# SpeakerGuard/SpeakerGuard

Hardware: AMD Instinct MI355X
Metric: PGD attack steps/sec (xv_plda, 3s@16kHz, batch 64) (higher is better)
Workload: dtype f32

## Files before the change

include/speakerguard_hip.h:

```cpp
#ifndef SPEAKERGUARD_HIP_H
#define SPEAKERGUARD_HIP_H

#include <stddef.h>
#include <stdint.h>

#ifdef __cplusplus
extern "C" {
#endif

typedef struct sg_ctx sg_ctx;

#define SG_OK 0
#define SG_ERR_ARG 1
#define SG_ERR_HIP 2
#define SG_ERR_STATE 3

int sg_version(void);
int sg_create(int device, sg_ctx** out);
void sg_destroy(sg_ctx* ctx);
const char* sg_last_error(const sg_ctx* ctx);
int sg_sync(sg_ctx* ctx, void* stream);
int sg_health(sg_ctx* ctx);
int sg_set_streamk(sg_ctx* ctx, int32_t enable);
int sg_debug_lose_handoffs(sg_ctx* ctx, int32_t launches);
// ... 136 lines not shown
} sg_an_weights;

int sg_an_load(sg_ctx* ctx, const sg_an_weights* w);
int32_t sg_an_num_frames(int32_t T);
int sg_an_logmel(sg_ctx* ctx, const float* x_dev, int32_t B, int32_t T, float* feats_dev, void* stream);
int sg_an_logmel_backward(sg_ctx* ctx, const float* x_dev, int32_t B, int32_t T, const float* dfeats_dev, float* grad_dev,
                          int32_t reuse_forward, void* stream);
int sg_an_configure(sg_ctx* ctx, int32_t fft_bits, int32_t spectrum_cache, int32_t fused_overlap_add);
int sg_an_forward(sg_ctx* ctx, const float* x_dev, int32_t B, int32_t T_or_F, int32_t flag,
                  int64_t* decisions_dev, float* scores_dev, float* emb_dev, void* stream);
int sg_an_debug_activation(sg_ctx* ctx, int32_t layer, float* out_dev, int64_t capacity_floats,
                           int32_t* rows_per_utt, int32_t* channels, void* stream);
int sg_an_loss_grad(sg_ctx* ctx, const float* x_dev, const int64_t* y_dev, int32_t B, int32_t T_or_F,
                    int32_t flag, const sg_loss_spec* loss, int64_t* decisions_dev, float* scores_dev,
                    float* loss_dev, float* grad_dev, void* stream);
int sg_an_pgd_run(sg_ctx* ctx, float* x_adv_dev, const int64_t* y_dev, const float* lower_dev,
                  const float* upper_dev, int32_t B, int32_t T, const sg_pgd_params* params,
                  uint8_t* success_dev, int64_t* decisions_dev, float* scores_dev, float* loss_dev,
                  float* loss_trace_dev, int64_t* decision_trace_dev, void* stream);

int sg_xv_time_layer(sg_ctx* ctx, int32_t layer, int32_t B, int32_t T, int32_t iters,
                     float* ms_per_launch, double* flops, int32_t* tile_rows, void* stream);

#define SG_STAGE_MFCC_FWD 10
#define SG_STAGE_CMVN_FWD 11
#define SG_STAGE_POOL_FWD 12
#define SG_STAGE_FC1_FWD 13
#define SG_STAGE_TAIL 14
#define SG_STAGE_FC1_BWD 15
#define SG_STAGE_POOL_BWD 16
#define SG_STAGE_CMVN_BWD 17
#define SG_STAGE_MFCC_BWD 18
#define SG_STAGE_OVERLAP_ADD 19
#define SG_STAGE_AN_LOGMEL_FWD 20
#define SG_STAGE_AN_PREFILTER_FWD 21
#define SG_STAGE_AN_POOL_FWD 22
#define SG_STAGE_AN_TAIL 23
#define SG_STAGE_AN_POOL_BWD 24
#define SG_STAGE_AN_PREFILTER_BWD 25
#define SG_STAGE_AN_LOGMEL_BWD 26
#define SG_STAGE_AN_OVERLAP_ADD 27
#define SG_STAGE_AN_FECO_FWD 28
#define SG_STAGE_AN_FECO_BWD 29
#define SG_STAGE_AN_CONV_FWD 30
#define SG_STAGE_AN_CONV_BWD 40
#define SG_STAGE_AN_FUSED_FWD 50
#define SG_STAGE_AN_FUSED_BWD 51
#define SG_STAGE_AN_FUSED_FWDBWD 52
int sg_trace_begin(sg_ctx* ctx, int32_t max_records);
int sg_trace_end(sg_ctx* ctx, int32_t* tags_out, float* ms_out, int32_t capacity, int32_t* n_out);

int sg_conv1d_rows(sg_ctx* ctx, const float* a_dev, const float* w_dev, float* c_dev, const float* bias_dev,
                   const float* mask_dev, int32_t B, int32_t Ta, int32_t Tc, int32_t Kc, int32_t N, int32_t taps,
                   int32_t tap_step, int32_t tap_base, int32_t epi, int32_t kernel, void* stream);

int sg_wav_finalize(sg_ctx* ctx, const float* benign_dev, const float* adver_dev, int32_t B, int32_t T,
                    int16_t* pcm_dev, double* metrics_dev, void* stream);

int sg_eer_threshold(sg_ctx* ctx, const float* target_dev, int32_t n_target, const float* untarget_dev,
                     int32_t n_untarget, double* out3_dev, void* stream);

int sg_feco_kmeans(sg_ctx* ctx, const float* feats_dev, int32_t B, int32_t F, int32_t D, int32_t k, int32_t max_iter,
                   int32_t* assign_dev, void* stream);
int sg_feco_kmeans_seeded(sg_ctx* ctx, const float* feats_dev, int32_t B, int32_t F, int32_t D, int32_t k, int32_t max_iter,
                          uint64_t seed, int64_t index_base, int32_t* assign_dev, void* stream);
int sg_feco_compress(sg_ctx* ctx, const float* feats_dev, const int32_t* assign_dev, int32_t B, int32_t F, int32_t D,
// ... 31 lines not shown
```

speakerguard_amd/_native.py:

```python
import ctypes as C
import os

_HERE = os.path.dirname(os.path.abspath(__file__))
LIB_PATH = os.path.join(_HERE, "libspeakerguard_hip.so")

SG_LOSS_ENTROPY, SG_LOSS_MARGIN, SG_LOSS_LINEAR = 0, 1, 2
SG_TASK = {"CSI": 0, "SV": 1, "OSI": 2}
SG_FLAG_WAV, SG_FLAG_RAW, SG_FLAG_CMVN = 0, 1, 2

EXPORTS = (
    "sg_version", "sg_create", "sg_destroy", "sg_last_error", "sg_sync", "sg_xv_load", "sg_xv_set_enroll",
    "sg_xv_num_frames", "sg_input_scale", "sg_xv_mfcc", "sg_xv_cmvn", "sg_xv_forward", "sg_xv_debug_activation",
    "sg_xv_loss_grad", "sg_loss_eval", "sg_pgd_update", "sg_xv_pgd_run", "sg_xv_time_layer",
    "sg_cw2_step", "sg_nes_queries", "sg_nes_grad", "sg_fakebob_step",
    "sg_an_load", "sg_an_num_frames", "sg_an_logmel", "sg_an_forward", "sg_an_debug_activation", "sg_an_loss_grad",
    "sg_an_pgd_run", "sg_an_pgd_run_feco", "sg_conv1d_rows", "sg_wav_finalize", "sg_eer_threshold",
    "sg_xv_mfcc_backward", "sg_xv_cmvn_backward", "sg_feco_kmeans", "sg_feco_kmeans_seeded", "sg_feco_kmeans_compress", "sg_feco_compress_backward_reps", "sg_feco_compress", "sg_feco_compress_backward", "sg_feco_warped",
    "sg_an_logmel_backward", "sg_an_configure", "sg_xv_configure", "sg_xv_enroll_override", "sg_health", "sg_set_streamk", "sg_debug_lose_handoffs", "sg_debug_feco_epoch", "sg_feco_set_two_cu", "sg_trace_begin", "sg_trace_end",
)

STAGE_NAMES = {10: "mfcc_fwd", 11: "cmvn_fwd", 12: "pool_fwd", 13: "fc1_fwd", 14: "tail", 15: "fc1_bwd", 16: "pool_bwd",
               17: "cmvn_bwd", 18: "mfcc_bwd", 19: "overlap_add"}
STAGE_NAMES.update({l: "tdnn%d_fwd" % l for l in range(1, 6)})
STAGE_NAMES.update({-l: "tdnn%d_dgrad" % l for l in range(1, 6)})
STAGE_NAMES.update({20: "an_logmel_fwd", 21: "an_prefilter_fwd", 22: "an_pool_fwd", 23: "an_tail", 24: "an_pool_bwd",
                    25: "an_prefilter_bwd", 26: "an_logmel_bwd", 27: "an_overlap_add", 28: "an_feco_fwd", 29: "an_feco_bwd",
                    50: "an_cnn_fwd", 51: "an_cnn_bwd", 52: "an_cnn_fwdbwd"})
STAGE_NAMES.update({30 + l: "an_conv%d_fwd" % (l + 2) for l in range(7)})
STAGE_NAMES.update({40 + l: "an_conv%d_dgrad" % (l + 2) for l in range(7)})


class NativeError(RuntimeError):
    pass


class XvWeights(C.Structure):
    _fields_ = [
        ("tdnn_weight", C.c_void_p * 5), ("tdnn_bias", C.c_void_p * 5),
        ("bn_mean", C.c_void_p * 5), ("bn_var", C.c_void_p * 5),
        ("fc1_weight", C.c_void_p), ("fc1_bias", C.c_void_p), ("emb_mean", C.c_void_p), ("lda", C.c_void_p),
        ("plda_mean", C.c_void_p), ("plda_transform", C.c_void_p), ("plda_psi", C.c_void_p), ("enroll", C.c_void_p),
        ("D", C.c_int32), ("S", C.c_int32), ("bn_eps", C.c_float), ("threshold", C.c_float),
    ]


class AnWeights(C.Structure):
    _fields_ = [
        ("conv1_weight", C.c_void_p), ("conv1_bias", C.c_void_p), ("bn1", C.c_void_p * 4),
        ("conv_weight", C.c_void_p * 7), ("conv_bias", C.c_void_p * 7), ("bn_weight", C.c_void_p * 7),
        ("bn_bias", C.c_void_p * 7), ("bn_mean", C.c_void_p * 7), ("bn_var", C.c_void_p * 7),
        ("fc_weight", C.c_void_p), ("fc_bias", C.c_void_p), ("num_class", C.c_int32), ("bn_eps", C.c_float),
    ]


class LossSpec(C.Structure):
# ... 137 lines not shown
```

speakerguard_amd/csrc/k_mfcc.hip:

```cpp
#include "sg_internal.h"
#include "fft512t.h"

namespace sg {

constexpr int kMfccMaxBlocks = 512;

template <typename R> struct MfccCfg;
#ifndef SG_MFCC_F32_WAVES
#define SG_MFCC_F32_WAVES 8
#define SG_MFCC_F32_OCC 4
#endif
template <> struct MfccCfg<float> { static constexpr int kWaves = SG_MFCC_F32_WAVES, kMinBlocks = SG_MFCC_F32_OCC; };
template <> struct MfccCfg<double> { static constexpr int kWaves = 4, kMinBlocks = 2; };

template <typename R>
struct FrameLdsT {
    cx<R> spec[kFft + kFft / 8];
    float power[256];
    float mel[32];
    float lmel[32];
    float tmp[32];
};

static_assert(kMfccTw1 == kFftTw1 && kMfccTw2 == kFftTw2, "table sizes of fft512.h");
// ... 168 lines not shown
        cep_out = v;
    }
}

template <typename R, int DZ>
__global__ __launch_bounds__(MfccCfg<R>::kWaves * 64, MfccCfg<R>::kMinBlocks) void mfcc_fwd_kernel(MfccTables t, const float* __restrict__ x, int B, int T, int F,
                                                                          const float* __restrict__ scale_p, sg_dither dz,
                                                                          float* __restrict__ feats) {
    constexpr int kWaves = MfccCfg<R>::kWaves;
    __shared__ FrameLdsT<R> lds[kWaves];
    __shared__ TabLdsT<R> tb;
    stage_tables<R>(t, tb);
    const int lane = threadIdx.x & 63, wid = threadIdx.x >> 6;
    const float scale = scale_p ? *scale_p : 1.f;
    FrameLdsT<R>& L = lds[wid];
    const int total = B * F, stride = gridDim.x * kWaves;
    float raw[7], nxt[7];
    load_frame(x, T, F, blockIdx.x * kWaves + wid, total, lane, nxt, t.rep_utts);
    for (int gf = blockIdx.x * kWaves + wid; gf < total; gf += stride) {
        const int b = gf / F, f = gf - b * F;
        const int tz = opaque_zero();
#pragma unroll
        for (int i = 0; i < 7; ++i) raw[i] = nxt[i];
        load_frame(x, T, F, gf + stride, total, lane, nxt, t.rep_utts);
        FrameState st;
        float cep;
        cx<R> Xk[4];
        frame_forward<R, 0, DZ>(t, tb, tz, L, raw, F, b, f, scale, dz, lane, st, cep, Xk);
        if (lane < kCep) feats[((size_t)b * F + f) * kCep + lane] = cep;
        wave_sync();
    }
}

template <typename R, bool CACHED, int DZ>
__global__ __launch_bounds__(MfccCfg<R>::kWaves * 64, CACHED ? MfccCfg<R>::kMinBlocks : 1) void mfcc_bwd_kernel(MfccTables t, const float* __restrict__ x, int B, int T, int F,
                                                                          const float* __restrict__ scale_p, sg_dither dz,
                                                                          const float* __restrict__ dfeats, int ld,
                                                                          float* __restrict__ dframes) {
    constexpr int kWaves = MfccCfg<R>::kWaves;
    __shared__ FrameLdsT<R> lds[kWaves];
    __shared__ TabLdsT<R> tb;
    stage_tables<R>(t, tb);
    const int lane = threadIdx.x & 63, wid = threadIdx.x >> 6;
    const float scale = scale_p ? *scale_p : 1.f;
    FrameLdsT<R>& L = lds[wid];
    const int kb = (lane >> 3) + 8 * (lane & 7);
    int bin_m0[4];
    float bin_w0[4], bin_w1[4];
#pragma unroll
    for (int d = 0; d < 4; ++d) {
        bin_m0[d] = t.bin_m0[kb + 64 * d];
        bin_w0[d] = t.bin_w0[kb + 64 * d];
        bin_w1[d] = t.bin_w1[kb + 64 * d];
    }
    const int total = B * F, stride = gridDim.x * kWaves;
    float raw[7], nxt[7];
    load_frame(x, T, F, blockIdx.x * kWaves + wid, total, lane, nxt, t.rep_utts);
    for (int gf = blockIdx.x * kWaves + wid; gf < total; gf += stride) {
        const int b = gf / F, f = gf - b * F;
        const int tz = opaque_zero();
#pragma unroll
        for (int i = 0; i < 7; ++i) raw[i] = nxt[i];
        load_frame(x, T, F, gf + stride, total, lane, nxt, t.rep_utts);
        FrameState st;
        float cep;
        cx<R> Xk[4];
        frame_forward<R, CACHED ? 1 : 0, DZ>(t, tb, tz, L, raw, F, b, f, scale, dz, lane, st, cep, Xk);
        float dc = 0.f;
        if (lane < kCep) dc = dfeats[((size_t)b * F + f) * ld + lane];
        const float denergy = __shfl(dc, 0, 64);
        if (lane < 32) L.tmp[lane] = (lane == 0 || lane >= kCep) ? 0.f : dc * tb.lifter[lane];
        wave_sync();
        if (lane < 32) {
            float dm = 0.f;
            if (lane < kMel) {
                float dl = 0.f;
#pragma unroll
                for (int c = 0; c < kCep; ++c) dl = __builtin_fmaf(L.tmp[c], tb.dct_t[tz + c * 32 + lane], dl);
                const float mel = L.mel[lane];
                dm = mel > kEps ? dl / mel : 0.f;
            }
            L.lmel[lane] = dm;
        }
        wave_sync();
        cx<R> v[8];
#pragma unroll
        for (int d = 0; d < 4; ++d) {
            v[d] = cmk<R>((R)0, (R)0);
            const int m0 = bin_m0[d];
            if (m0 >= 0) {
                const R dp = (R)(2.f * __builtin_fmaf(L.lmel[m0], bin_w0[d], L.lmel[m0 + 1] * bin_w1[d]));
                v[d] = cmk<R>(Xk[d].x * dp, Xk[d].y * dp);
            }
        }
#pragma unroll
        for (int d = 4; d < 8; ++d) v[d] = cmk<R>((R)0, (R)0);
        fft512T_transposed<R>(L.spec, tb.tw1c() + tz, tb.tw2c() + tz, lane, (R)1, v);
        float sw[8];
#pragma unroll
        for (int i = 0; i < 7; ++i) sw[i] = (float)v[i].x * tb.window[tz + lane + 64 * i];
        sw[7] = 0.f;
        float ds[7];
        float sum = 0.f;
        const float einv = st.energy > kEps ? 2.f * denergy / st.energy : 0.f;
#pragma unroll
        for (int i = 0; i < 7; ++i) {
            const int n = lane + 64 * i;
            const float edge = __builtin_bit_cast(float, __builtin_amdgcn_readlane(__builtin_bit_cast(int, sw[i + 1]), 0));
            const float next = __builtin_bit_cast(float, __builtin_amdgcn_update_dpp(__builtin_bit_cast(int, edge), __builtin_bit_cast(int, sw[i]),
                                                                                      0x130 , 0xf, 0xf, false));
            float g = 0.f;
            if (n < kWin) {
                g = sw[i] - 0.97f * next;
                if (n == 0) g -= 0.97f * sw[0];
                g = __builtin_fmaf(einv, st.s[i], g);
            }
            ds[i] = g;
            sum += g;
        }
        const float mean = wave_sum(sum) / (float)kWin;
#pragma unroll
        for (int i = 0; i < 7; ++i) {
            const int n = lane + 64 * i;
            if (n < kWin) dframes[((size_t)b * F + f) * kWin + n] = (ds[i] - mean) * scale;
        }
        wave_sync();
    }
}
#pragma clang fp contract(fast)

template <int V>
__global__ __launch_bounds__(256) void frames_to_wave_kernel(const float* __restrict__ dframes, int B, int T, int F, int R,
                                                             const float* acc_in, float* grad_out, float* __restrict__ x_io,
                                                             const float* __restrict__ lower,
                                                             const float* __restrict__ upper, float step, int grad_sign) {
    const int n0 = (blockIdx.x * 256 + threadIdx.x) * V;
    const int b = blockIdx.y;
    if (n0 >= T) return;
    constexpr int kPad = kWin / 2 - kShift / 2;
    const int last_q = (F - 1) * kShift - kPad + kWin - 1;
    const size_t o = (size_t)b * T + n0;
    float total[V];
    const bool interior = V == 4 && n0 >= kPad && 2 * T - 1 - (n0 + 3) > last_q && n0 + 3 < T;
    if (interior) {
        typedef float f4 __attribute__((ext_vector_type(4)));
        const int q = n0 + kPad;
        int fhi = q / kShift;
        const int flo = q > kWin - 1 ? (q - (kWin - 1) + kShift - 1) / kShift : 0;
        if (fhi > F - 1) fhi = F - 1;
        f4 tot = {0.f, 0.f, 0.f, 0.f};
        for (int r = 0; r < R; ++r) {
            const float* df = dframes + ((size_t)r * B + b) * F * kWin;
            f4 g = {0.f, 0.f, 0.f, 0.f};
            for (int f = flo; f <= fhi; ++f) g += *reinterpret_cast<const f4*>(df + (size_t)f * kWin + (q - f * kShift));
            if (r == 0) tot = acc_in ? *reinterpret_cast<const f4*>(acc_in + o) + g : g;
            else tot = tot + g;
        }
// ... 25 lines not shown
        }
    }
    if (V == 4 && n0 + 3 < T) {
        typedef float f4 __attribute__((ext_vector_type(4)));
        if (grad_out) *reinterpret_cast<f4*>(grad_out + o) = f4{total[0], total[V > 1 ? 1 : 0], total[V > 2 ? 2 : 0], total[V > 3 ? 3 : 0]};
        if (x_io) {
            const f4 xv = *reinterpret_cast<const f4*>(x_io + o), lo = *reinterpret_cast<const f4*>(lower + o),
                     hi = *reinterpret_cast<const f4*>(upper + o);
            f4 res;
#pragma unroll
            for (int v = 0; v < 4; ++v) {
                const float g = total[v < V ? v : 0];
                const float sg = g > 0.f ? 1.f : (g < 0.f ? -1.f : 0.f);
                res[v] = fminf(fmaxf(xv[v] + step * sg * (float)grad_sign, lo[v]), hi[v]);
            }
            *reinterpret_cast<f4*>(x_io + o) = res;
        }
        return;
    }
#pragma unroll
    for (int v = 0; v < V; ++v) {
        if (n0 + v >= T) break;
        const float g = total[v];
        if (grad_out) grad_out[o + v] = g;
        if (x_io) {
            const float sg = g > 0.f ? 1.f : (g < 0.f ? -1.f : 0.f);
            float val = x_io[o + v] + step * sg * (float)grad_sign;
            val = fminf(fmaxf(val, lower[o + v]), upper[o + v]);
            x_io[o + v] = val;
        }
    }
}

template <typename R>
static void mfcc_fwd_launch(const MfccTables& t, const float* x, int B, int T, int F, const float* scale, const sg_dither& d,
                            float* feats, hipStream_t s) {
    constexpr int kWaves = MfccCfg<R>::kWaves;
    const int want = (B * F + kWaves - 1) / kWaves;
    dim3 grid(want < kMfccMaxBlocks ? want : kMfccMaxBlocks);
    if (d.noise_dev) hipLaunchKernelGGL((mfcc_fwd_kernel<R, 2>), grid, dim3(kWaves * 64), 0, s, t, x, B, T, F, scale, d, feats);
    else if (d.dither != 0.f) hipLaunchKernelGGL((mfcc_fwd_kernel<R, 1>), grid, dim3(kWaves * 64), 0, s, t, x, B, T, F, scale, d, feats);
    else hipLaunchKernelGGL((mfcc_fwd_kernel<R, 0>), grid, dim3(kWaves * 64), 0, s, t, x, B, T, F, scale, d, feats);
}

template <typename R>
static void mfcc_bwd_launch(const MfccTables& t, const float* x, int B, int T, int F, const float* scale, const sg_dither& d,
                            const float* dfeats, float* dframes, hipStream_t s) {
    constexpr int kWaves = MfccCfg<R>::kWaves;
    const int want = (B * F + kWaves - 1) / kWaves;
    dim3 grid(want < kMfccMaxBlocks ? want : kMfccMaxBlocks);
#define SG_MFCC_BWD(CACHED, DZ) \
    hipLaunchKernelGGL((mfcc_bwd_kernel<R, CACHED, DZ>), grid, dim3(kWaves * 64), 0, s, t, x, B, T, F, scale, d, dfeats, kCep, dframes)
    const int dzk = d.noise_dev ? 2 : (d.dither != 0.f ? 1 : 0);
    if (t.spec_cache) {
        if (dzk == 2) SG_MFCC_BWD(true, 2); else if (dzk == 1) SG_MFCC_BWD(true, 1); else SG_MFCC_BWD(true, 0);
    } else {
        if (dzk == 2) SG_MFCC_BWD(false, 2); else if (dzk == 1) SG_MFCC_BWD(false, 1); else SG_MFCC_BWD(false, 0);
    }
#undef SG_MFCC_BWD
}

hipError_t launch_mfcc_fwd(const MfccTables& t, const float* x, int B, int T, int F, const float* scale,
                           const sg_dither* dz, float* feats, hipStream_t s) {
    sg_dither d = dz ? *dz : sg_dither{0.f, 0, 0, nullptr};
    if (t.fft64) mfcc_fwd_launch<double>(t, x, B, T, F, scale, d, feats, s);
    else mfcc_fwd_launch<float>(t, x, B, T, F, scale, d, feats, s);
    return hipGetLastError();
}

hipError_t launch_mfcc_bwd(const MfccTables& t, const float* x, int B, int T, int F, const float* scale,
                           const sg_dither* dz, const float* dfeats, float* dframes, hipStream_t s) {
    sg_dither d = dz ? *dz : sg_dither{0.f, 0, 0, nullptr};
    if (t.fft64) mfcc_bwd_launch<double>(t, x, B, T, F, scale, d, dfeats, dframes, s);
    else mfcc_bwd_launch<float>(t, x, B, T, F, scale, d, dfeats, dframes, s);
    return hipGetLastError();
}

hipError_t launch_frames_to_wave(const float* dframes, int B, int T, int F, int R, const float* acc_in, float* grad_out,
                                 float* x_io, const float* lower, const float* upper, float step, int grad_sign,
                                 hipStream_t s) {
    const uintptr_t bases = reinterpret_cast<uintptr_t>(grad_out) | reinterpret_cast<uintptr_t>(x_io) |
                            reinterpret_cast<uintptr_t>(lower) | reinterpret_cast<uintptr_t>(upper) |
                            reinterpret_cast<uintptr_t>(acc_in) | reinterpret_cast<uintptr_t>(dframes);
    if (T % 4 == 0 && bases % 16 == 0 && (long)B * T >= 16L * 48000) {
        dim3 grid((T / 4 + 255) / 256, B);
        hipLaunchKernelGGL(frames_to_wave_kernel<4>, grid, dim3(256), 0, s, dframes, B, T, F, R, acc_in, grad_out, x_io, lower, upper,
                           step, grad_sign);
    } else {
        dim3 grid((T + 255) / 256, B);
        hipLaunchKernelGGL(frames_to_wave_kernel<1>, grid, dim3(256), 0, s, dframes, B, T, F, R, acc_in, grad_out, x_io, lower, upper,
                           step, grad_sign);
    }
    return hipGetLastError();
}

}
```

speakerguard_amd/csrc/sg_api.hip:

```cpp
#include <algorithm>
#include <cmath>
#include <cstdarg>
#include <cstdio>
#include <cstdlib>
#include <cstring>
#include <memory>
#include <type_traits>

#include "sg_internal.h"

using namespace sg;

namespace {

int fail(sg_ctx* ctx, int code, const char* fmt, ...) {
    char buf[512];
    va_list ap;
    va_start(ap, fmt);
    vsnprintf(buf, sizeof(buf), fmt, ap);
    va_end(ap);
    if (ctx) ctx->err = buf;
    return code;
}

// ... 343 lines not shown
    if (int h = sg_health(ctx)) return h;
    SG_HIP(hipSetDevice(ctx->device));
    if (B < 1) return fail(ctx, SG_ERR_ARG, "B must be >= 1");
    if (flag < 0 || flag > 2) return fail(ctx, SG_ERR_ARG, "flag must be 0 (wav), 1 (raw feat) or 2 (cmvn feat)");
    d->B = B;
    if (flag == SG_FLAG_WAV) {
        if (TF < kWin) return fail(ctx, SG_ERR_ARG, "waveform shorter than one 25 ms window");
        d->T = TF;
        d->F = num_frames(TF);
    } else {
        d->T = 0;
        d->F = TF;
    }
    int Fl[kLayers];
    if (!layer_frames(d->F, Fl)) return fail(ctx, SG_ERR_ARG, "%d frames are too few for the TDNN context", d->F);
    {
        size_t worst = 0;
        for (int l = 0; l < kLayers; ++l) {
            const size_t bytes = (size_t)B * Fl[l] * kCoutPad[l] * sizeof(float);
            if (bytes > worst) worst = bytes;
        }
        if (worst >= 0x80000000ull)
            return fail(ctx, SG_ERR_ARG, "batch of %d x %d frames needs a %.1f GiB activation tensor; one pass handles < 2 GiB "
                        "(at most %d utterances of this length): split the batch", B, d->F, (double)worst / (1ull << 30),
                        (int)(0x7FFFFFFFull / (worst / (size_t)B)));
    }
    int rc = build_tables(ctx);
    if (rc) return rc;
    rc = ensure_workspace(ctx, d->B, d->T, d->F);
    if (rc) return fail(ctx, rc, "workspace allocation failed: %s", ctx->err.c_str());
    return SG_OK;
}

int run_backward_to_input(sg_ctx* ctx, const float* x, const PassDims& d, int flag, const sg_dither* dz,
                          float* grad_out, float* x_update, const float* lower, const float* upper, float step,
                          int grad_sign, hipStream_t s, const float* grad_acc_in = nullptr) {
    Workspace& w = ctx->ws;
    int rc = run_tdnn_backward(ctx, d, s);
    if (rc) return rc;
    if (flag == SG_FLAG_CMVN) {
        SG_HIP(launch_sum_cols(w.dfeats, kFeatPad, kL1BwdSplitK, (long long)d.B * d.F * kFeatPad, grad_out, kCep,
                               (int64_t)d.B * d.F, kCep, s));
    } else if (flag == SG_FLAG_RAW) {
        SG_HIP(launch_cmvn_bwd(w.dfeats, kFeatPad, kL1BwdSplitK, (long long)d.B * d.F * kFeatPad, grad_out, kCep, d.B,
                               d.F, s));
    } else {
        SG_STAGE(SG_STAGE_CMVN_BWD, launch_cmvn_bwd(w.dfeats, kFeatPad, kL1BwdSplitK, (long long)d.B * d.F * kFeatPad,
                                                    w.dfeats_raw, kCep, d.B, d.F, s));
        MfccTables tab = ctx->tab;
        static const bool use_cache = [] {
            const char* e = sg_tune_env("SG_MFCC_CACHE");
            return !e || atoi(e) != 0;
        }();
        if (use_cache) {
            tab.spec_cache = w.spec_cache;
            tab.mel_cache = w.mel_cache;
        }
        tab.rep_utts = d.Bu;
        const int utts = d.Bu > 0 ? d.Bu : d.B;
        SG_STAGE(SG_STAGE_MFCC_BWD, launch_mfcc_bwd(tab, x, d.B, d.T, d.F, w.scale, dz, w.dfeats_raw, w.dframes, s));
        SG_STAGE(SG_STAGE_OVERLAP_ADD, launch_frames_to_wave(w.dframes, utts, d.T, d.F, d.B / utts, grad_acc_in, grad_out, x_update,
                                                             lower, upper, step, grad_sign, s));
    }
    return SG_OK;
}

}

extern "C" {

int sg_version(void) { return 100; }

int sg_create(int device, sg_ctx** out) {
    if (!out) return SG_ERR_ARG;
    *out = nullptr;
    int n = 0;
    if (hipGetDeviceCount(&n) != hipSuccess || device < 0 || device >= n) return SG_ERR_HIP;
    if (hipSetDevice(device) != hipSuccess) return SG_ERR_HIP;
    sg_ctx* ctx = new (std::nothrow) sg_ctx();
    if (!ctx) return SG_ERR_HIP;
    ctx->device = device;
    hipDeviceProp_t prop;
    if (hipGetDeviceProperties(&prop, device) == hipSuccess && prop.multiProcessorCount > 0)
        ctx->num_cus = prop.multiProcessorCount;
    if (hipEventCreate(&ctx->ev0) != hipSuccess || hipEventCreate(&ctx->ev1) != hipSuccess) {
        delete ctx;
        return SG_ERR_HIP;
// ... 413 lines not shown
        const int F = num_frames(T);
        if (!layer_frames(F, Fl)) return fail(ctx, SG_ERR_ARG, "%d frames are too few for the TDNN context", F);
        size_t per_utt = 0;
        for (int l = 0; l < kLayers; ++l) per_utt = std::max(per_utt, (size_t)Fl[l] * kCoutPad[l] * sizeof(float));
        long max_rows = (long)(0x7FFFFFFFull / per_utt);
        if (const char* e = sg_tune_env("SG_EOT_MAX_ROWS")) max_rows = std::min<long>(max_rows, atol(e));
        G = (int)std::min<long>(reps, std::max<long>(1, max_rows / B));
    }
    PassDims d;
    rc = check_dims(ctx, B * G, T, SG_FLAG_WAV, &d);
    if (rc) return rc;
    Workspace& w = ctx->ws;
    for (int r = 0; r < G; ++r)
        SG_HIP(hipMemcpyAsync(w.y_rep + (size_t)r * B, y_dev, (size_t)B * sizeof(int64_t), hipMemcpyDeviceToDevice, s));
    const bool want_rec = loss_trace_dev || decision_trace_dev;
    if (want_rec && G < reps && w.eot_rows_cap < (size_t)reps * B) {
        if (w.eot_loss_rows || w.eot_dec_rows) {
            SG_HIP(hipStreamSynchronize(s));
            for (void* old : {static_cast<void*>(w.eot_loss_rows), static_cast<void*>(w.eot_dec_rows)}) {
                auto it = std::find(w.allocs.begin(), w.allocs.end(), old);
                if (it != w.allocs.end()) {
                    (void)hipFree(old);
                    w.allocs.erase(it);
                }
            }
            w.eot_loss_rows = nullptr;
            w.eot_dec_rows = nullptr;
            w.eot_rows_cap = 0;
        }
        if ((rc = dev_alloc(ctx, w.allocs, &w.eot_loss_rows, (size_t)reps * B))) return rc;
        if ((rc = dev_alloc(ctx, w.allocs, &w.eot_dec_rows, (size_t)reps * B))) return rc;
        w.eot_rows_cap = (size_t)reps * B;
    }
    for (int it = 0; it <= p->max_iter; ++it) {
        const bool last = it == p->max_iter;
        const int nrep = last ? 1 : reps;
        for (int g0 = 0; g0 < nrep; g0 += G) {
            const int Gi = std::min(G, nrep - g0);
            sg_dither dz = p->dither;
            dz.seed += (uint64_t)it * 0x9E3779B97F4A7C15ull + (uint64_t)g0 * 0xC2B2AE3D27D4EB4Full;
            d.B = B * Gi;
            d.Bu = Gi > 1 ? B : 0;
            d.keep_scale = it > 0 || g0 > 0;
            if ((rc = run_frontend(ctx, x_adv_dev, d, SG_FLAG_WAV, &dz, !last, s))) return rc;
            if ((rc = run_tdnn_forward(ctx, d, s))) return rc;
            TailArgs t{};
            t.fc1_part = w.fc1_part; t.nsplit = kFc1SplitK; t.B = d.B; t.m = &ctx->xv; t.y = w.y_rep; t.loss = p->loss;
            t.want_grad = !last; t.demb = w.demb;
            t.scores = last ? scores_dev : nullptr;
            t.decisions = last ? decisions_dev : nullptr;
            t.loss_out = last ? loss_dev : nullptr;
            t.success = last ? success_dev : nullptr;
            const bool direct = nrep == 1, grouped = nrep > G;
            float* lrows = grouped ? w.eot_loss_rows + (size_t)g0 * B : w.loss;
            int64_t* drows = grouped ? w.eot_dec_rows + (size_t)g0 * B : w.decisions;
            t.loss_trace = !want_rec ? nullptr : (direct && loss_trace_dev ? loss_trace_dev + (size_t)it * B : lrows);
            t.decision_trace = !want_rec ? nullptr : (direct && decision_trace_dev ? decision_trace_dev + (size_t)it * B : drows);
            t.coef_rows = B;
            SG_STAGE(SG_STAGE_TAIL, launch_tail(t, s));
            if (want_rec && !direct && g0 + Gi >= nrep)
                SG_HIP(launch_eot_trace_reduce(grouped ? w.eot_loss_rows : w.loss, grouped ? w.eot_dec_rows : w.decisions, nrep, B,
                                               loss_trace_dev ? loss_trace_dev + (size_t)it * B : nullptr,
                                               decision_trace_dev ? decision_trace_dev + (size_t)it * B : nullptr, s));
            if (!last) {
                const bool final_group = g0 + Gi >= nrep;
                rc = run_backward_to_input(ctx, x_adv_dev, d, SG_FLAG_WAV, &dz, final_group ? nullptr : w.grad,
                                           final_group ? x_adv_dev : nullptr, lower_dev, upper_dev, p->step_size, p->grad_sign, s,
                                           g0 > 0 ? w.grad : nullptr);
                if (rc) return rc;
            }
        }
    }
    return SG_OK;
}

int sg_trace_begin(sg_ctx* ctx, int32_t max_records) {
    if (!ctx) return SG_ERR_ARG;
    if (max_records < 1 || max_records > (1 << 20)) return fail(ctx, SG_ERR_ARG, "max_records must be 1 .. 2^20");
    SG_HIP(hipSetDevice(ctx->device));
    while ((int)ctx->trace_ev.size() < 2 * max_records) {
        hipEvent_t e = nullptr;
        SG_HIP(hipEventCreate(&e));
        ctx->trace_ev.push_back(e);
    }
    ctx->trace_tag.assign((size_t)max_records, 0);
    ctx->trace_used = 0;
    ctx->trace_open = false;
    ctx->trace_dropped = 0;
    ctx->trace_on = true;
    return SG_OK;
}

int sg_trace_end(sg_ctx* ctx, int32_t* tags_out, float* ms_out, int32_t capacity, int32_t* n_out) {
    if (!ctx || !n_out) return SG_ERR_ARG;
    if (!ctx->trace_on) return fail(ctx, SG_ERR_STATE, "sg_trace_end without sg_trace_begin");
    ctx->trace_on = false;
    ctx->trace_open = false;
    const int n = ctx->trace_used;
    *n_out = n;
    if (ctx->trace_dropped)
        return fail(ctx, SG_ERR_HIP, "stage trace: %d event record(s) failed, %d launch records kept", ctx->trace_dropped, n);
    if (n > 0) SG_HIP(hipEventSynchronize(ctx->trace_ev[2 * (n - 1) + 1]));
    for (int i = 0; i < n && i < capacity; ++i) {
        float ms = 0.f;
        SG_HIP(hipEventElapsedTime(&ms, ctx->trace_ev[2 * i], ctx->trace_ev[2 * i + 1]));
// ... 77 lines not shown
```

speakerguard_amd/csrc/sg_internal.h:

```cpp
#pragma once
#include <hip/hip_runtime.h>
#include <cstdlib>
#include <stdint.h>
#include <string>
#include <vector>

#include "../../include/speakerguard_hip.h"

namespace sg {

constexpr int kShift = 160;
constexpr int kWin = 400;
constexpr int kFft = 512;
constexpr int kMel = 30;
constexpr int kCep = 30;
constexpr int kLdaLd = 516;
constexpr int kFeatPad = 32;
constexpr int kCmnWindow = 300;
constexpr float kEps = 1.1920928955078125e-07f;

constexpr int kLayers = 5;
constexpr int kCin[kLayers] = {30, 512, 512, 512, 512};
constexpr int kCout[kLayers] = {512, 512, 512, 512, 1500};
constexpr int kCinPad[kLayers] = {32, 512, 512, 512, 512};
// ... 158 lines not shown
    int enroll_cap = 0;
    const float* enroll_override = nullptr;
    int S_override = 0;
    std::vector<void*> allocs;
};

struct Workspace {
    int B = 0, T = 0, F = 0;
    int Fl[kLayers] = {};
    float* scale = nullptr;
    float* feats_raw = nullptr;
    float* feats = nullptr;
    float* act[kLayers] = {};
    float* dact[kLayers] = {};
    float* dfeats = nullptr;
    float* dfeats_raw = nullptr;
    float* dframes = nullptr;
    float2* spec_cache = nullptr;
    float* mel_cache = nullptr;
    float* stats = nullptr;
    float* fc1_part = nullptr;
    float* demb = nullptr;
    float* dstats_part = nullptr;
    float* tdnn_emb = nullptr;
    float* emb = nullptr;
    float* scores = nullptr;
    float* loss = nullptr;
    int64_t* decisions = nullptr;
    float* grad = nullptr;
    int64_t* y_rep = nullptr;
    float* eot_loss_rows = nullptr;
    int64_t* eot_dec_rows = nullptr;
    size_t eot_rows_cap = 0;
    std::vector<void*> allocs;
};

}

struct sg_ctx {
    int device = 0;
    int num_cus = 256;
    std::string err;
    sg::MfccTables tab{};
    bool tables_ready = false;
    float* range_scratch = nullptr;
    float* cw2_scratch = nullptr;
    float* sk_slabs = nullptr;
    unsigned* sk_flags = nullptr;
    sg::XvModel xv;
    sg::Workspace ws;
    unsigned* err_host = nullptr;
    unsigned* err_dev = nullptr;
    bool use_streamk = true;
    int lose_handoffs = 0;
    int lose_feco = 0;
    unsigned long long* feco_xchg = nullptr;
    unsigned* feco_flags = nullptr;
    unsigned feco_epoch = 0;
    int feco_two_cu = -1;
    sg::AnTables an_tab{};
    sg::AnFrontCfg an_cfg{};
    bool an_tables_ready = false;
    sg::AnModel an;
    sg::AnWorkspace an_ws;
    std::vector<void*> model_allocs;
    hipEvent_t ev0 = nullptr, ev1 = nullptr;
// ... 73 lines not shown
        const int d = sg_device_slot();
        if (cap[d] < bytes) {
            if (ptr[d]) (void)hipFree(ptr[d]);
            ptr[d] = nullptr;
            cap[d] = 0;
            if (hipMalloc(&ptr[d], bytes) == hipSuccess) cap[d] = bytes;
        }
        return ptr[d];
    }
};

inline void conv_ctx_args(sg_ctx* ctx, ConvGemmArgs& a) {
    a.sk_slabs = ctx->sk_slabs;
    a.sk_flags = ctx->sk_flags;
    a.err_word = ctx->err_dev;
    a.num_cus = ctx->num_cus;
    a.no_streamk = ctx->use_streamk ? 0 : 1;
    a.ablate = 0;
    a.lose_counter = ctx->use_streamk ? &ctx->lose_handoffs : nullptr;
}

hipError_t launch_conv_gemm(const ConvGemmArgs& a, int tile, int epi, int splits, hipStream_t s);
int conv_gemm_tile_rows(int M, int N);
hipError_t launch_pack_k4(const float* w, int K, int N, float* wq, hipStream_t s);

hipError_t launch_input_scale(const float* x, int64_t n, float* scratch512, float* scale, int mode, hipStream_t s);
hipError_t launch_mfcc_fwd(const MfccTables& t, const float* x, int B, int T, int F, const float* scale,
                           const sg_dither* dz, float* feats, hipStream_t s);
hipError_t launch_mfcc_bwd(const MfccTables& t, const float* x, int B, int T, int F, const float* scale,
                           const sg_dither* dz, const float* dfeats, float* dframes, hipStream_t s);
hipError_t launch_frames_to_wave(const float* dframes, int B, int T, int F, int R, const float* acc_in, float* grad_out,
                                 float* x_io, const float* lower, const float* upper, float step, int grad_sign,
                                 hipStream_t s);
hipError_t launch_pgd_update(float* x, const float* g, const float* lo, const float* hi, int64_t n,
                             float step, int grad_sign, hipStream_t s);
hipError_t launch_copy_cols(const float* in, int ld_in, float* out, int ld_out, int64_t rows, int ncol, hipStream_t s);
hipError_t launch_sum_cols(const float* in, int ld_in, int nsplit, long long slab_stride, float* out, int ld_out,
                           int64_t rows, int ncol, hipStream_t s);
hipError_t launch_cmvn_fwd(const float* in, int ld_in, float* out, int ld_out, int B, int F, hipStream_t s);
hipError_t launch_cmvn_bwd(const float* dout, int ld_dout, int nsplit, long long slab_stride, float* din, int ld_din,
                           int B, int F, hipStream_t s);
hipError_t launch_pool_fwd(const float* act5, int B, int Tc, float* stats, hipStream_t s);
hipError_t launch_pool_bwd(const float* act5, const float* stats, const float* dstats_part, int nsplit,
                           int B, int Tc, float* dact5, hipStream_t s);

hipError_t launch_cw2_step(float* modifier, float* exp_avg, float* exp_avg_sq, const float* x, const float* input_cur,
                           const float* grad1, const float* const_c, int B, int T, float lr, int step_t,
                           float* input_next, float* loss2, float* scratch, hipStream_t s);
hipError_t launch_nes_queries(const float* x, int n, int T, int half, int with_clean, float sigma, uint64_t seed,
                              int64_t index_base, int pair_base, const float* noise_in, float* queries, float* noise_out,
                              hipStream_t s);
hipError_t launch_nes_grad(const float* loss, int n, int T, int half, int with_clean, uint64_t seed, int64_t index_base,
                           int pair_base, const float* noise_in, int accumulate, float final_sigma, int final_batches,
                           float* grad, hipStream_t s);
hipError_t launch_fakebob_step(float* x, float* grad, const float* prev_grad, const float* lr, const float* lower,
                               const float* upper, int n, int T, float momentum, float one_m_momentum, int grad_sign,
                               hipStream_t s);

hipError_t launch_loss_eval(const float* scores, const int64_t* y, int B, int S, float threshold, const sg_loss_spec& ls,
                            int64_t* dec, float* loss, float* dscores, hipStream_t s);
hipError_t launch_eot_trace_reduce(const float* loss_rows, const int64_t* dec_rows, int R, int B, float* loss_out,
                                   int64_t* dec_out, hipStream_t s);

struct AnHeadArgs {
    int on;
    const float* fc_w;
// ... 61 lines not shown
```

Measured before the change: 407.1.

## Fuse MFCC backward, overlap-add PGD update and next-step MFCC forward into one seam kernel

Adds a seam kernel that, per utterance slab, runs the MFCC adjoint (including recomputed halo frames so no cross-block handoff is needed), overlap-adds the frame gradients, applies the sign-step PGD update with clamping, and immediately recomputes the next iteration's MFCC features and spectral caches. The next iteration then only runs CMVN forward instead of the full frontend. This removes separate mfcc_bwd, frames_to_wave and mfcc_fwd launches and their global round trips. In exchange it adds ping-pong buffers for x and caches, redundant halo frame work, a grid limited to about one block per CU-slab, and a final device copy when x ends up in the alternate buffer.

```diff
diff --git a/include/speakerguard_hip.h b/include/speakerguard_hip.h
--- a/include/speakerguard_hip.h
+++ b/include/speakerguard_hip.h
@@ -192,6 +192,7 @@
 #define SG_STAGE_CMVN_BWD 17
 #define SG_STAGE_MFCC_BWD 18
 #define SG_STAGE_OVERLAP_ADD 19
+#define SG_STAGE_MFCC_SEAM 60
 #define SG_STAGE_AN_LOGMEL_FWD 20
 #define SG_STAGE_AN_PREFILTER_FWD 21
 #define SG_STAGE_AN_POOL_FWD 22
diff --git a/speakerguard_amd/_native.py b/speakerguard_amd/_native.py
--- a/speakerguard_amd/_native.py
+++ b/speakerguard_amd/_native.py
@@ -20,7 +20,7 @@
 )
 
 STAGE_NAMES = {10: "mfcc_fwd", 11: "cmvn_fwd", 12: "pool_fwd", 13: "fc1_fwd", 14: "tail", 15: "fc1_bwd", 16: "pool_bwd",
-               17: "cmvn_bwd", 18: "mfcc_bwd", 19: "overlap_add"}
+               17: "cmvn_bwd", 18: "mfcc_bwd", 19: "overlap_add", 60: "mfcc_seam"}
 STAGE_NAMES.update({l: "tdnn%d_fwd" % l for l in range(1, 6)})
 STAGE_NAMES.update({-l: "tdnn%d_dgrad" % l for l in range(1, 6)})
 STAGE_NAMES.update({20: "an_logmel_fwd", 21: "an_prefilter_fwd", 22: "an_pool_fwd", 23: "an_tail", 24: "an_pool_bwd",
diff --git a/speakerguard_amd/csrc/k_mfcc.hip b/speakerguard_amd/csrc/k_mfcc.hip
--- a/speakerguard_amd/csrc/k_mfcc.hip
+++ b/speakerguard_amd/csrc/k_mfcc.hip
@@ -224,6 +224,81 @@
     }
 }
 
+struct BinLane {
+    int m0[4];
+    float w0[4], w1[4];
+};
+__device__ __forceinline__ void load_bin_lane(const MfccTables& t, int lane, BinLane& bl) {
+    const int kb = (lane >> 3) + 8 * (lane & 7);
+#pragma unroll
+    for (int d = 0; d < 4; ++d) {
+        bl.m0[d] = t.bin_m0[kb + 64 * d];
+        bl.w0[d] = t.bin_w0[kb + 64 * d];
+        bl.w1[d] = t.bin_w1[kb + 64 * d];
+    }
+}
+
+template <typename R>
+__device__ __forceinline__ void frame_adjoint(const TabLdsT<R>& tb, int tz, FrameLdsT<R>& L, const BinLane& bl,
+                                              const float* __restrict__ dfeats, size_t gfi, int ld, float scale, int lane,
+                                              const FrameState& st, const cx<R> (&Xk)[4], float (&out)[7]) {
+    float dc = 0.f;
+    if (lane < kCep) dc = dfeats[gfi * ld + lane];
+    const float denergy = __shfl(dc, 0, 64);
+    if (lane < 32) L.tmp[lane] = (lane == 0 || lane >= kCep) ? 0.f : dc * tb.lifter[lane];
+    wave_sync();
+    if (lane < 32) {
+        float dm = 0.f;
+        if (lane < kMel) {
+            float dl = 0.f;
+#pragma unroll
+            for (int c = 0; c < kCep; ++c) dl = __builtin_fmaf(L.tmp[c], tb.dct_t[tz + c * 32 + lane], dl);
+            const float mel = L.mel[lane];
+            dm = mel > kEps ? dl / mel : 0.f;
+        }
+        L.lmel[lane] = dm;
+    }
+    wave_sync();
+    cx<R> v[8];
+#pragma unroll
+    for (int d = 0; d < 4; ++d) {
+        v[d] = cmk<R>((R)0, (R)0);
+        const int m0 = bl.m0[d];
+        if (m0 >= 0) {
+            const R dp = (R)(2.f * __builtin_fmaf(L.lmel[m0], bl.w0[d], L.lmel[m0 + 1] * bl.w1[d]));
+            v[d] = cmk<R>(Xk[d].x * dp, Xk[d].y * dp);
+        }
+    }
+#pragma unroll
+    for (int d = 4; d < 8; ++d) v[d] = cmk<R>((R)0, (R)0);
+    fft512T_transposed<R>(L.spec, tb.tw1c() + tz, tb.tw2c() + tz, lane, (R)1, v);
+    float sw[8];
+#pragma unroll
+    for (int i = 0; i < 7; ++i) sw[i] = (float)v[i].x * tb.window[tz + lane + 64 * i];
+    sw[7] = 0.f;
+    float ds[7];
+    float sum = 0.f;
+    const float einv = st.energy > kEps ? 2.f * denergy / st.energy : 0.f;
+#pragma unroll
+    for (int i = 0; i < 7; ++i) {
+        const int n = lane + 64 * i;
+        const float edge = __builtin_bit_cast(float, __builtin_amdgcn_readlane(__builtin_bit_cast(int, sw[i + 1]), 0));
+        const float next = __builtin_bit_cast(float, __builtin_amdgcn_update_dpp(__builtin_bit_cast(int, edge), __builtin_bit_cast(int, sw[i]),
+                                                                                  0x130 , 0xf, 0xf, false));
+        float g = 0.f;
+        if (n < kWin) {
+            g = sw[i] - 0.97f * next;
+            if (n == 0) g -= 0.97f * sw[0];
+            g = __builtin_fmaf(einv, st.s[i], g);
+        }
+        ds[i] = g;
+        sum += g;
+    }
+    const float mean = wave_sum(sum) / (float)kWin;
+#pragma unroll
+    for (int i = 0; i < 7; ++i) out[i] = (ds[i] - mean) * scale;
+}
+
 template <typename R, bool CACHED, int DZ>
 __global__ __launch_bounds__(MfccCfg<R>::kWaves * 64, CACHED ? MfccCfg<R>::kMinBlocks : 1) void mfcc_bwd_kernel(MfccTables t, const float* __restrict__ x, int B, int T, int F,
                                                                           const float* __restrict__ scale_p, sg_dither dz,
@@ -236,15 +311,8 @@
     const int lane = threadIdx.x & 63, wid = threadIdx.x >> 6;
     const float scale = scale_p ? *scale_p : 1.f;
     FrameLdsT<R>& L = lds[wid];
-    const int kb = (lane >> 3) + 8 * (lane & 7);
-    int bin_m0[4];
-    float bin_w0[4], bin_w1[4];
-#pragma unroll
-    for (int d = 0; d < 4; ++d) {
-        bin_m0[d] = t.bin_m0[kb + 64 * d];
-        bin_w0[d] = t.bin_w0[kb + 64 * d];
-        bin_w1[d] = t.bin_w1[kb + 64 * d];
-    }
+    BinLane bl;
+    load_bin_lane(t, lane, bl);
     const int total = B * F, stride = gridDim.x * kWaves;
     float raw[7], nxt[7];
     load_frame(x, T, F, blockIdx.x * kWaves + wid, total, lane, nxt, t.rep_utts);
@@ -258,63 +326,12 @@
         float cep;
         cx<R> Xk[4];
         frame_forward<R, CACHED ? 1 : 0, DZ>(t, tb, tz, L, raw, F, b, f, scale, dz, lane, st, cep, Xk);
-        float dc = 0.f;
-        if (lane < kCep) dc = dfeats[((size_t)b * F + f) * ld + lane];
-        const float denergy = __shfl(dc, 0, 64);
-        if (lane < 32) L.tmp[lane] = (lane == 0 || lane >= kCep) ? 0.f : dc * tb.lifter[lane];
-        wave_sync();
-        if (lane < 32) {
-            float dm = 0.f;
-            if (lane < kMel) {
-                float dl = 0.f;
-#pragma unroll
-                for (int c = 0; c < kCep; ++c) dl = __builtin_fmaf(L.tmp[c], tb.dct_t[tz + c * 32 + lane], dl);
-                const float mel = L.mel[lane];
-                dm = mel > kEps ? dl / mel : 0.f;
-            }
-            L.lmel[lane] = dm;
-        }
-        wave_sync();
-        cx<R> v[8];
-#pragma unroll
-        for (int d = 0; d < 4; ++d) {
-            v[d] = cmk<R>((R)0, (R)0);
-            const int m0 = bin_m0[d];
-            if (m0 >= 0) {
-                const R dp = (R)(2.f * __builtin_fmaf(L.lmel[m0], bin_w0[d], L.lmel[m0 + 1] * bin_w1[d]));
-                v[d] = cmk<R>(Xk[d].x * dp, Xk[d].y * dp);
-            }
-        }
-#pragma unroll
-        for (int d = 4; d < 8; ++d) v[d] = cmk<R>((R)0, (R)0);
-        fft512T_transposed<R>(L.spec, tb.tw1c() + tz, tb.tw2c() + tz, lane, (R)1, v);
-        float sw[8];
-#pragma unroll
-        for (int i = 0; i < 7; ++i) sw[i] = (float)v[i].x * tb.window[tz + lane + 64 * i];
-        sw[7] = 0.f;
-        float ds[7];
-        float sum = 0.f;
-        const float einv = st.energy > kEps ? 2.f * denergy / st.energy : 0.f;
+        float g[7];
+        frame_adjoint<R>(tb, tz, L, bl, dfeats, (size_t)b * F + f, ld, scale, lane, st, Xk, g);
 #pragma unroll
         for (int i = 0; i < 7; ++i) {
             const int n = lane + 64 * i;
-            const float edge = __builtin_bit_cast(float, __builtin_amdgcn_readlane(__builtin_bit_cast(int, sw[i + 1]), 0));
-            const float next = __builtin_bit_cast(float, __builtin_amdgcn_update_dpp(__builtin_bit_cast(int, edge), __builtin_bit_cast(int, sw[i]),
-                                                                                      0x130 , 0xf, 0xf, false));
-            float g = 0.f;
-            if (n < kWin) {
-                g = sw[i] - 0.97f * next;
-                if (n == 0) g -= 0.97f * sw[0];
-                g = __builtin_fmaf(einv, st.s[i], g);
-            }
-            ds[i] = g;
-            sum += g;
-        }
-        const float mean = wave_sum(sum) / (float)kWin;
-#pragma unroll
-        for (int i = 0; i < 7; ++i) {
-            const int n = lane + 64 * i;
-            if (n < kWin) dframes[((size_t)b * F + f) * kWin + n] = (ds[i] - mean) * scale;
+            if (n < kWin) dframes[((size_t)b * F + f) * kWin + n] = g[i];
         }
         wave_sync();
     }
@@ -406,6 +423,114 @@
     }
 }
 
+constexpr int kSeamHalo = 2;
+constexpr int kSeamTail = kWin - kShift;
+constexpr int kSeamWaves = 16;
+template <typename R>
+__global__ __launch_bounds__(kSeamWaves * 64, 1) void mfcc_seam_kernel(
+    MfccTables t, const float* __restrict__ x, float* x_out, int T, int F, int S, const float* __restrict__ scale_p,
+    const float* __restrict__ dfeats, float* dframes, float* halo, const float* __restrict__ lower,
+    const float* __restrict__ upper, float step, int grad_sign, float2* __restrict__ spec_out, float* __restrict__ mel_out,
+    float* __restrict__ feats) {
+    constexpr int kWaves = kSeamWaves;
+    constexpr int kPad = kWin / 2 - kShift / 2;
+    __shared__ FrameLdsT<R> lds[kWaves];
+    __shared__ TabLdsT<R> tb;
+    __shared__ float xtail[kSeamTail];
+    stage_tables<R>(t, tb);
+    const int lane = threadIdx.x & 63, wid = threadIdx.x >> 6;
+    const float scale = *scale_p;
+    FrameLdsT<R>& L = lds[wid];
+    const int b = blockIdx.y, f0 = blockIdx.x * S, f1 = min(F, f0 + S);
+    const int h0 = max(0, f0 - kSeamHalo), h1 = min(F, f1 + kSeamHalo);
+    float* hrows = halo + ((size_t)b * gridDim.x + blockIdx.x) * (2 * kSeamHalo) * kWin;
+    auto frame_row = [&](int f) -> float* {
+        if (f >= f0 && f < f1) return dframes + ((size_t)b * F + f) * kWin;
+        return hrows + (f < f0 ? f - (f0 - kSeamHalo) : kSeamHalo + f - f1) * kWin;
+    };
+    const sg_dither dz0{0.f, 0, 0, nullptr};
+    {
+        BinLane bl;
+        load_bin_lane(t, lane, bl);
+        float raw[7], nxt[7];
+        if (h0 + wid < h1) load_frame(x, T, F, b * F + h0 + wid, b * F + h1, lane, nxt, 0);
+        for (int f = h0 + wid; f < h1; f += kWaves) {
+            const int tz = opaque_zero();
+#pragma unroll
+            for (int i = 0; i < 7; ++i) raw[i] = nxt[i];
+            load_frame(x, T, F, b * F + f + kWaves, b * F + h1, lane, nxt, 0);
+            FrameState st;
+            float cep;
+            cx<R> Xk[4];
+            frame_forward<R, 1, 0>(t, tb, tz, L, raw, F, b, f, scale, dz0, lane, st, cep, Xk);
+            float g[7];
+            frame_adjoint<R>(tb, tz, L, bl, dfeats, (size_t)b * F + f, kCep, scale, lane, st, Xk, g);
+            float* row = frame_row(f);
+#pragma unroll
+            for (int i = 0; i < 7; ++i) {
+                const int n = lane + 64 * i;
+                if (n < kWin) row[n] = g[i];
+            }
+            wave_sync();
+        }
+    }
+    __syncthreads();
+    const int lo = f0 == 0 ? 0 : f0 * kShift - kPad;
+    const int hi = min(T, f1 * kShift + kPad);
+    const int own_hi = f1 == F ? T : f1 * kShift - kPad;
+    {
+        const int last_q = (F - 1) * kShift - kPad + kWin - 1;
+        for (int n = lo + (int)threadIdx.x; n < hi; n += blockDim.x) {
+            const int pr = 2 * T - 1 - n;
+            float g = 0.f;
+            auto add_pos = [&](int p) {
+                const int q = p + kPad;
+                int fhi = q / kShift;
+                const int flo = q > kWin - 1 ? (q - (kWin - 1) + kShift - 1) / kShift : 0;
+                if (fhi > F - 1) fhi = F - 1;
+                for (int f = flo; f <= fhi; ++f) g += frame_row(f)[q - f * kShift];
+            };
+            add_pos(n);
+            if (n < kPad) add_pos(-n - 1);
+            if (pr <= last_q) add_pos(pr);
+            const size_t o = (size_t)b * T + n;
+            const float sg = g > 0.f ? 1.f : (g < 0.f ? -1.f : 0.f);
+            float val = x[o] + step * sg * (float)grad_sign;
+            val = fminf(fmaxf(val, lower[o]), upper[o]);
+            if (n < own_hi) x_out[o] = val;
+            else xtail[n - own_hi] = val;
+        }
+    }
+    __syncthreads();
+    MfccTables tn = t;
+    tn.spec_cache = spec_out;
+    tn.mel_cache = mel_out;
+    auto load_new = [&](int f, float (&raw)[7]) {
+        const int base = f * kShift - kPad;
+#pragma unroll
+        for (int i = 0; i < 7; ++i) {
+            const int n = lane + 64 * i;
+            const int p = base + (n < kWin ? n : kWin - 1);
+            const int idx = p < 0 ? -p - 1 : (p >= T ? 2 * T - 1 - p : p);
+            raw[i] = idx < own_hi ? x_out[(size_t)b * T + idx] : xtail[idx - own_hi];
+        }
+    };
+    float raw[7], nxt[7];
+    if (f0 + wid < f1) load_new(f0 + wid, nxt);
+    for (int f = f0 + wid; f < f1; f += kWaves) {
+        const int tz = opaque_zero();
+#pragma unroll
+        for (int i = 0; i < 7; ++i) raw[i] = nxt[i];
+        if (f + kWaves < f1) load_new(f + kWaves, nxt);
+        FrameState st;
+        float cep;
+        cx<R> Xk[4];
+        frame_forward<R, 0, 0>(tn, tb, tz, L, raw, F, b, f, scale, dz0, lane, st, cep, Xk);
+        if (lane < kCep) feats[((size_t)b * F + f) * kCep + lane] = cep;
+        wave_sync();
+    }
+}
+
 template <typename R>
 static void mfcc_fwd_launch(const MfccTables& t, const float* x, int B, int T, int F, const float* scale, const sg_dither& d,
                             float* feats, hipStream_t s) {
@@ -447,6 +572,19 @@
     sg_dither d = dz ? *dz : sg_dither{0.f, 0, 0, nullptr};
     if (t.fft64) mfcc_bwd_launch<double>(t, x, B, T, F, scale, d, dfeats, dframes, s);
     else mfcc_bwd_launch<float>(t, x, B, T, F, scale, d, dfeats, dframes, s);
+    return hipGetLastError();
+}
+
+int mfcc_seam_slabs(int F, int S) { return (F + S - 1) / S; }
+
+hipError_t launch_mfcc_seam(const MfccTables& t, const float* x, float* x_out, int B, int T, int F, int S, const float* scale,
+                            const float* dfeats, float* dframes, float* halo, const float* lower, const float* upper,
+                            float step, int grad_sign, float2* spec_out, float* mel_out, float* feats, hipStream_t s) {
+    if (t.fft64 || !t.spec_cache || !t.mel_cache || t.rep_utts != 0 || S < 1 || x == x_out || t.spec_cache == spec_out)
+        return hipErrorInvalidValue;
+    dim3 grid(mfcc_seam_slabs(F, S), B);
+    hipLaunchKernelGGL(mfcc_seam_kernel<float>, grid, dim3(kSeamWaves * 64), 0, s, t, x, x_out, T, F, S, scale, dfeats, dframes,
+                       halo, lower, upper, step, grad_sign, spec_out, mel_out, feats);
     return hipGetLastError();
 }
 
diff --git a/speakerguard_amd/csrc/sg_api.hip b/speakerguard_amd/csrc/sg_api.hip
--- a/speakerguard_amd/csrc/sg_api.hip
+++ b/speakerguard_amd/csrc/sg_api.hip
@@ -399,9 +399,66 @@
     return SG_OK;
 }
 
+bool mfcc_cache_on() {
+    static const bool on = [] {
+        const char* e = sg_tune_env("SG_MFCC_CACHE");
+        return !e || atoi(e) != 0;
+    }();
+    return on;
+}
+
+bool mfcc_seam_on() {
+    const char* e = sg_tune_env("SG_MFCC_SEAM");
+    return !e || atoi(e) != 0;
+}
+
+int mfcc_seam_slab(const sg_ctx* ctx, int B, int F) {
+    if (const char* e = sg_tune_env("SG_MFCC_SEAM_S")) {
+        const int v = atoi(e);
+        if (v >= 1) return v;
+    }
+    const int slabs = std::max(1, ctx->num_cus / B);
+    return (F + slabs - 1) / slabs;
+}
+
+struct SeamStep {
+    float* x_out;
+    float2* spec_out;
+    float* mel_out;
+    const float2* spec_in;
+    const float* mel_in;
+    int S;
+};
+
+int ensure_seam_buffers(sg_ctx* ctx, int B, int T, int F, int S, hipStream_t s) {
+    Workspace& w = ctx->ws;
+    const size_t nx = (size_t)B * T, nf = (size_t)B * F, nh = (size_t)B * mfcc_seam_slabs(F, S) * 4 * kWin;
+    if (nx <= w.seam_x_cap && nf <= w.seam_frames_cap && nh <= w.seam_halo_cap) return SG_OK;
+    SG_HIP(hipStreamSynchronize(s));
+    for (void* old : {static_cast<void*>(w.x_alt), static_cast<void*>(w.spec_cache2), static_cast<void*>(w.mel_cache2),
+                      static_cast<void*>(w.seam_halo)}) {
+        auto it = std::find(w.allocs.begin(), w.allocs.end(), old);
+        if (old && it != w.allocs.end()) {
+            (void)hipFree(old);
+            w.allocs.erase(it);
+        }
+    }
+    w.x_alt = nullptr; w.spec_cache2 = nullptr; w.mel_cache2 = nullptr; w.seam_halo = nullptr;
+    w.seam_x_cap = w.seam_frames_cap = w.seam_halo_cap = 0;
+    int rc = 0;
+    const size_t cx_ = std::max(nx, (size_t)w.B * w.T), cf = std::max(nf, (size_t)w.B * w.F);
+    rc |= dev_alloc(ctx, w.allocs, &w.x_alt, cx_);
+    rc |= dev_alloc(ctx, w.allocs, &w.spec_cache2, cf * 256);
+    rc |= dev_alloc(ctx, w.allocs, &w.mel_cache2, cf * 32);
+    rc |= dev_alloc(ctx, w.allocs, &w.seam_halo, nh);
+    if (rc) return fail(ctx, SG_ERR_HIP, "seam workspace allocation failed");
+    w.seam_x_cap = cx_; w.seam_frames_cap = cf; w.seam_halo_cap = nh;
+    return SG_OK;
+}
+
 int run_backward_to_input(sg_ctx* ctx, const float* x, const PassDims& d, int flag, const sg_dither* dz,
                           float* grad_out, float* x_update, const float* lower, const float* upper, float step,
-                          int grad_sign, hipStream_t s, const float* grad_acc_in = nullptr) {
+                          int grad_sign, hipStream_t s, const float* grad_acc_in = nullptr, const SeamStep* seam = nullptr) {
     Workspace& w = ctx->ws;
     int rc = run_tdnn_backward(ctx, d, s);
     if (rc) return rc;
@@ -415,11 +472,16 @@
         SG_STAGE(SG_STAGE_CMVN_BWD, launch_cmvn_bwd(w.dfeats, kFeatPad, kL1BwdSplitK, (long long)d.B * d.F * kFeatPad,
                                                     w.dfeats_raw, kCep, d.B, d.F, s));
         MfccTables tab = ctx->tab;
-        static const bool use_cache = [] {
-            const char* e = sg_tune_env("SG_MFCC_CACHE");
-            return !e || atoi(e) != 0;
-        }();
-        if (use_cache) {
+        if (seam) {
+            tab.spec_cache = const_cast<float2*>(seam->spec_in);
+            tab.mel_cache = const_cast<float*>(seam->mel_in);
+            tab.rep_utts = 0;
+            SG_STAGE(SG_STAGE_MFCC_SEAM, launch_mfcc_seam(tab, x, seam->x_out, d.B, d.T, d.F, seam->S, w.scale, w.dfeats_raw,
+                                                          w.dframes, w.seam_halo, lower, upper, step, grad_sign,
+                                                          seam->spec_out, seam->mel_out, w.feats_raw, s));
+            return SG_OK;
+        }
+        if (mfcc_cache_on()) {
             tab.spec_cache = w.spec_cache;
             tab.mel_cache = w.mel_cache;
         }
@@ -899,6 +961,13 @@
         if ((rc = dev_alloc(ctx, w.allocs, &w.eot_dec_rows, (size_t)reps * B))) return rc;
         w.eot_rows_cap = (size_t)reps * B;
     }
+    const bool seam = reps == 1 && p->dither.dither == 0.f && !p->dither.noise_dev && !ctx->tab.fft64 && mfcc_cache_on() &&
+                      p->max_iter > 0 && mfcc_seam_on();
+    const int seam_S = seam ? mfcc_seam_slab(ctx, B, d.F) : 0;
+    if (seam && (rc = ensure_seam_buffers(ctx, B, T, d.F, seam_S, s))) return rc;
+    float* xc = x_adv_dev;
+    float2* spec_c = w.spec_cache;
+    float* mel_c = w.mel_cache;
     for (int it = 0; it <= p->max_iter; ++it) {
         const bool last = it == p->max_iter;
         const int nrep = last ? 1 : reps;
@@ -909,7 +978,8 @@
             d.B = B * Gi;
             d.Bu = Gi > 1 ? B : 0;
             d.keep_scale = it > 0 || g0 > 0;
-            if ((rc = run_frontend(ctx, x_adv_dev, d, SG_FLAG_WAV, &dz, !last, s))) return rc;
+            if (seam && it > 0) SG_STAGE(SG_STAGE_CMVN_FWD, launch_cmvn_fwd(w.feats_raw, kCep, w.feats, kFeatPad, d.B, d.F, s));
+            else if ((rc = run_frontend(ctx, x_adv_dev, d, SG_FLAG_WAV, &dz, !last, s))) return rc;
             if ((rc = run_tdnn_forward(ctx, d, s))) return rc;
             TailArgs t{};
             t.fc1_part = w.fc1_part; t.nsplit = kFc1SplitK; t.B = d.B; t.m = &ctx->xv; t.y = w.y_rep; t.loss = p->loss;
@@ -929,7 +999,23 @@
                 SG_HIP(launch_eot_trace_reduce(grouped ? w.eot_loss_rows : w.loss, grouped ? w.eot_dec_rows : w.decisions, nrep, B,
                                                loss_trace_dev ? loss_trace_dev + (size_t)it * B : nullptr,
                                                decision_trace_dev ? decision_trace_dev + (size_t)it * B : nullptr, s));
-            if (!last) {
+            if (!last && seam) {
+                SeamStep st;
+                const bool first = xc == x_adv_dev;
+                const bool next_last = it + 1 == p->max_iter;
+                st.x_out = first ? w.x_alt : x_adv_dev;
+                st.spec_in = spec_c;
+                st.mel_in = mel_c;
+                st.spec_out = next_last ? nullptr : (spec_c == w.spec_cache ? w.spec_cache2 : w.spec_cache);
+                st.mel_out = next_last ? nullptr : (mel_c == w.mel_cache ? w.mel_cache2 : w.mel_cache);
+                st.S = seam_S;
+                if ((rc = run_backward_to_input(ctx, xc, d, SG_FLAG_WAV, &dz, nullptr, nullptr, lower_dev, upper_dev, p->step_size,
+                                                p->grad_sign, s, nullptr, &st)))
+                    return rc;
+                xc = st.x_out;
+                spec_c = st.spec_out;
+                mel_c = st.mel_out;
+            } else if (!last) {
                 const bool final_group = g0 + Gi >= nrep;
                 rc = run_backward_to_input(ctx, x_adv_dev, d, SG_FLAG_WAV, &dz, final_group ? nullptr : w.grad,
                                            final_group ? x_adv_dev : nullptr, lower_dev, upper_dev, p->step_size, p->grad_sign, s,
@@ -938,6 +1024,7 @@
             }
         }
     }
+    if (xc != x_adv_dev) SG_HIP(hipMemcpyAsync(x_adv_dev, xc, (size_t)B * T * sizeof(float), hipMemcpyDeviceToDevice, s));
     return SG_OK;
 }
 
diff --git a/speakerguard_amd/csrc/sg_internal.h b/speakerguard_amd/csrc/sg_internal.h
--- a/speakerguard_amd/csrc/sg_internal.h
+++ b/speakerguard_amd/csrc/sg_internal.h
@@ -214,6 +214,11 @@
     float* eot_loss_rows = nullptr;
     int64_t* eot_dec_rows = nullptr;
     size_t eot_rows_cap = 0;
+    float* x_alt = nullptr;
+    float2* spec_cache2 = nullptr;
+    float* mel_cache2 = nullptr;
+    float* seam_halo = nullptr;
+    size_t seam_x_cap = 0, seam_frames_cap = 0, seam_halo_cap = 0;
     std::vector<void*> allocs;
 };
 
@@ -353,6 +358,10 @@
 hipError_t launch_frames_to_wave(const float* dframes, int B, int T, int F, int R, const float* acc_in, float* grad_out,
                                  float* x_io, const float* lower, const float* upper, float step, int grad_sign,
                                  hipStream_t s);
+int mfcc_seam_slabs(int F, int S);
+hipError_t launch_mfcc_seam(const MfccTables& t, const float* x, float* x_out, int B, int T, int F, int S, const float* scale,
+                            const float* dfeats, float* dframes, float* halo, const float* lower, const float* upper,
+                            float step, int grad_sign, float2* spec_out, float* mel_out, float* feats, hipStream_t s);
 hipError_t launch_pgd_update(float* x, const float* g, const float* lo, const float* hi, int64_t n,
                              float step, int grad_sign, hipStream_t s);
 hipError_t launch_copy_cols(const float* in, int ld_in, float* out, int ld_out, int64_t rows, int ncol, hipStream_t s);
```

After: 407.2 (median of 6 runs). No clear change (+0.0%).
